# bifurcation/fourq

Hardware: AMD Instinct MI355X
Metric: FourQ scalar-mults/sec (batch, whole node) (higher is better)
Workload: dtype u64

## Files before the change

fourq_amd/build.py:

```python
import json
import os
import re
import shutil
import subprocess
import sys

HERE = os.path.dirname(os.path.abspath(__file__))
SRC_DIR = os.path.join(HERE, "csrc")
LIB_PATH = os.path.join(HERE, "libfourq_amd.so")
RESOURCES_PATH = os.path.join(HERE, "kernel_resources.json")
PLACEMENT_PATH = os.path.join(HERE, "code_placement.json")
SOURCES = ["fourq_amd.hip", "fourq_chain.hip", "fourq_ct_fused.hip", "fourq_ct_chain.hip"]
HEADERS = ["fp127.hip.h", "curve.hip.h", "recode.hip.h", "kernels.hip.h", "pair.hip.h", "ladder_asm.hip.h", "ladder_asm_gfx950.inc", "constants.inc", "pipeline_plan.h", os.path.join("..", "..", "include", "fourq_amd.h")]
HIPCC_FLAGS = ["-O3", "--offload-arch=gfx950", "-std=c++17", "-fPIC", "-fvisibility=hidden", "-Rpass-analysis=kernel-resource-usage"]
PLACE_TOOL = os.path.normpath(os.path.join(HERE, "..", "tools", "asmgen", "place_asm.py"))
LLVM_BIN = "/opt/rocm/lib/llvm/bin"
BUNDLE_TARGETS = "host-x86_64-unknown-linux-gnu,hipv4-amdgcn-amd-amdhsa--gfx950"
BUNDLE_COMPRESS = [] if os.environ.get("FOURQ_BUILD_NO_COMPRESS") == "1" else ["--compress"]

RESOURCE_POLICY = [
    (r"ladder_kernel<\d, 2,", "scratch", lambda v: v == 0, "the two-kernel route's ladders must not spill"),
    (r"ladder_kernel<\d, 2, true", "occupancy", lambda v: v >= 4, "the two-kernel route's DH ladders are sized for 4 waves per SIMD (128 VGPRs)"),
    (r"ladder_kernel<\d, 2, false", "occupancy", lambda v: v >= 2, "the two-kernel route's MUL ladders run the asm bodies at 2 waves per SIMD"),
    (r"ladder_kernel<\d, 1, \w+, \w+, false>", "scratch", lambda v: v == 0, "the fixed-base ladders (MUL and DH) must not spill"),
    (r"ladder_kernel<\d, 1, \w+, \w+, false>", "occupancy", lambda v: v >= 2, "the fixed-base ladders run the asm bodies at 2 waves per SIMD"),
    (r"ladder_kernel<\d, 1, \w+, \w+, true>", "scratch", lambda v: v == 0, "the constant-time fixed-base ladders must not spill"),
    (r"ladder_kernel<\d, 0,", "scratch", lambda v: v == 0, "the fused variable-base kernels must not spill to memory (AGPR copies are fine)"),
    (r"pair_kernel<", "scratch", lambda v: v == 0, "the two-lanes-per-element kernel must not spill"),
    (r"prep_kernel<0, \w+>\(", "occupancy", lambda v: v >= 2, "prep_kernel<ENDO> hides its read-backs behind a second wave per SIMD"),
    (r"mixed_ct_tail_kernel<", "occupancy", lambda v: v >= 2, "the constant-time mixed-batch tail runs the asm bodies at two waves per SIMD"),
    (r"mixed_ct_tail_kernel<", "scratch", lambda v: v == 0, "the constant-time mixed-batch tail must not spill"),
    (r"comb_kernel<true, false>", "scratch", lambda v: v == 0, "the keygen comb of large batches (deferred normalisation) must not touch scratch memory"),
    (r"comb_kernel<false, false>", "scratch", lambda v: v <= 16, "the keygen comb with its inversion in the kernel parks 4 registers around the call: no more than that"),
]


def _hipcc():
    exe = shutil.which("hipcc") or "/opt/rocm/bin/hipcc"
    if not os.path.exists(exe):
        raise RuntimeError("hipcc not found: the FourQ engine needs the ROCm toolchain to build")
    return exe


def _demangle(names):
    filt = shutil.which("c++filt") or "/opt/rocm/lib/llvm/bin/llvm-cxxfilt"
    try:
        out = subprocess.run([filt], input="\n".join(names), capture_output=True, text=True, check=True).stdout.splitlines()
        return [o.replace("fq::(anonymous namespace)::", "").replace("(anonymous namespace)::", "") for o in out]
    except (OSError, subprocess.CalledProcessError):
        return list(names)


_FIELDS = {"TotalSGPRs": "sgprs", "VGPRs": "vgprs", "AGPRs": "agprs", "ScratchSize [bytes/lane]": "scratch",
           "Occupancy [waves/SIMD]": "occupancy", "VGPRs Spill": "vgpr_spills", "SGPRs Spill": "sgpr_spills", "LDS Size [bytes/block]": "lds"}


def parse_resource_remarks(text):
    kernels, cur = {}, None
    for line in text.splitlines():
        m = re.search(r"remark:\s+(Function Name|[A-Za-z ]+(?:\[[^\]]+\])?):\s*(\S+)\s*\[-Rpass-analysis", line)
        if not m:
            continue
        key, val = m.group(1).strip(), m.group(2)
        if key == "Function Name":
            cur = kernels.setdefault(val, {})
        elif cur is not None and key in _FIELDS:
            try:
                cur[_FIELDS[key]] = int(val)
            except ValueError:
                pass
    return kernels


def check_policy(resources):
    bad = []
    for unit, kernels in resources.items():
        for name, f in kernels.items():
            for pattern, field, ok, why in RESOURCE_POLICY:
                if re.search(pattern, name) and field in f and not ok(f[field]):
                    bad.append("%s: %s has %s = %d (%s)" % (unit, name, field, f[field], why))
    return bad


def source_id(extra_flags=()):
    import hashlib
    h = hashlib.sha256()
    for f in [os.path.join(SRC_DIR, f) for f in SOURCES + HEADERS] + [PLACE_TOOL]:
        with open(os.path.normpath(f), "rb") as fh:
            h.update(fh.read())
    h.update(" ".join(list(HIPCC_FLAGS) + list(extra_flags)).encode())
    return h.hexdigest()[:16]


def is_stale():
    if not os.path.exists(LIB_PATH):
        return True
    built = os.path.getmtime(LIB_PATH)
    deps = [os.path.join(SRC_DIR, f) for f in SOURCES + HEADERS] + [PLACE_TOOL]
    return any(os.path.getmtime(os.path.normpath(d)) > built for d in deps)


FASTCODEC_SRC = os.path.join(SRC_DIR, "fastcodec.c")


def fastcodec_path():
    import sysconfig
    return os.path.join(HERE, "_fastcodec" + sysconfig.get_config_var("EXT_SUFFIX"))


def build_fastcodec(force=False, verbose=False):
    import sysconfig
    out = fastcodec_path()
    if not force and os.path.exists(out) and os.path.getmtime(out) >= os.path.getmtime(FASTCODEC_SRC):
        return out
    cc = shutil.which("gcc") or shutil.which("cc")
    if cc is None:
        raise RuntimeError("no C compiler for fourq_amd/csrc/fastcodec.c")
    _run([cc, "-O2", "-shared", "-fPIC", "-Wall", "-I" + sysconfig.get_paths()["include"], "-o", out, FASTCODEC_SRC], verbose)
    return out


def _run(cmd, verbose=False):
    if verbose:
        print(" ".join(cmd), file=sys.stderr)
    proc = subprocess.run(cmd, stdout=subprocess.PIPE, stderr=subprocess.STDOUT, text=True)
    if proc.returncode != 0:
        raise RuntimeError("command failed: %s\n%s" % (" ".join(cmd), "\n".join(l for l in proc.stdout.splitlines() if "remark:" not in l)[-6000:]))
    return proc.stdout


class RegisterOwnershipError(Exception):
    """A kernel reaches a hand-scheduled body whose physical registers lie outside its allocation.  NOT a RuntimeError on purpose: the
    build's fallback for a failed placement detour catches RuntimeError, and this finding must never be swallowed by it -- the plain
    hipcc build of the same sources would carry the same kernel."""


def check_register_ranges(asm_path):
    kernel, highest, alloc, accum = None, {}, {}, {}
    with open(asm_path) as fh:
        for ln in fh:
            m = re.match(r"^(_Z\w+):", ln)
            if m:
                kernel = m.group(1)
                continue
            m = re.match(r"\s*\.amdhsa_kernel\s+(\S+)", ln)
            if m:
                kernel = m.group(1)
                continue
            m = re.match(r"\s*\.amdhsa_next_free_vgpr\s+(\d+)", ln)
            if m and kernel:
                alloc[kernel] = int(m.group(1))
                continue
            m = re.match(r"\s*\.amdhsa_accum_offset\s+(\d+)", ln)
            if m and kernel:
                accum[kernel] = int(m.group(1))
                continue
            t = ln.strip()
            if kernel is None or not t or t[0] in ";.":
                continue
            for a, b in re.findall(r"\bv(\d+)\b|\bv\[\d+:(\d+)\]", t):
                r = int(a or b)
                if r > highest.get(kernel, -1):
                    highest[kernel] = r
    bad = []
    for k, h in highest.items():
        if k not in alloc:
            continue
        owned = min(alloc[k], accum.get(k, alloc[k]))
        if h >= owned:
            bad.append("%s names v%d but owns %d arch VGPRs (next_free_vgpr %d, accum_offset %s)" % (k, h, owned, alloc[k], accum.get(k, "-")))
    if not alloc and highest:
        bad.append("%s: VGPRs are named but no .amdhsa_next_free_vgpr could be parsed -- the listing format changed" % asm_path)
    if bad:
        raise RegisterOwnershipError("a kernel reaches an asm body whose registers it does not own:\n  " + "\n  ".join(bad))


def compile_unit(src, obj, flags, verbose=False, place=True, placement=None):
    src_path = os.path.join(SRC_DIR, src)
    stem = os.path.splitext(obj)[0]
    if not place:
        if placement is not None:
            placement[src] = {"placed": False}
        listing = stem + ".check.s"
        try:
            _run([_hipcc()] + [f for f in flags if not f.startswith("-Rpass")] + ["--cuda-device-only", "-S", "-o", listing, src_path], verbose)
            check_register_ranges(listing)
        finally:
            if os.path.exists(listing):
                os.remove(listing)
        return _run([_hipcc()] + flags + ["-c", "-o", obj, src_path], verbose)
    import importlib.util
    spec = importlib.util.spec_from_file_location("place_asm", PLACE_TOOL)
    place_asm = importlib.util.module_from_spec(spec)
    spec.loader.exec_module(place_asm)
    dev_s, placed_s, dev_o, hsaco, fatbin = stem + ".dev.s", stem + ".placed.s", stem + ".dev.o", stem + ".hsaco", stem + ".hipfb"
    remarks = _run([_hipcc()] + flags + ["--cuda-device-only", "-S", "-o", dev_s, src_path], verbose)
    check_register_ranges(dev_s)
    stats = place_asm.place_file(dev_s, placed_s)
    if placement is not None:
        placement[src] = {"placed": True, "wide_instructions": stats["wide_total"], "at_4_mod_8_before": stats["misaligned_before"],
                          "at_4_mod_8_after": stats["misaligned_after"], "reencoded": stats["promoted"], "nops": stats["nops"],
                          "instructions_compared_with_the_unplaced_object": stats["instructions_compared"]}
    if verbose:
        print("%s: %d of %d 8-byte instructions at 4 mod 8 before placement, %d after" % (
            src, stats["misaligned_before"], stats["wide_total"], stats["misaligned_after"]), file=sys.stderr)
    _run([os.path.join(LLVM_BIN, "clang"), "-x", "assembler", "-target", "amdgcn-amd-amdhsa", "-mcpu=gfx950", "-c", placed_s, "-o", dev_o], verbose)
    _run([os.path.join(LLVM_BIN, "lld"), "-flavor", "gnu", "-m", "elf64_amdgpu", "--no-undefined", "-shared", "-o", hsaco, dev_o], verbose)
    _run([os.path.join(LLVM_BIN, "clang-offload-bundler"), "-type=o", "-bundle-align=4096", "-targets=" + BUNDLE_TARGETS] + BUNDLE_COMPRESS +
         ["-input=/dev/null", "-input=" + hsaco, "-output=" + fatbin], verbose)
    host_flags = [f for f in flags if not f.startswith("-Rpass")]
    _run([_hipcc()] + host_flags + ["--cuda-host-only", "-Xclang", "-fcuda-include-gpubinary", "-Xclang", fatbin, "-c", "-o", obj, src_path], verbose)
    for tmp in (dev_s, placed_s, dev_o, hsaco, fatbin):
        os.remove(tmp)
    return remarks


def build_library(force=False, verbose=False, extra_flags=(), out_path=None):
    if out_path is None:
        try:
            build_fastcodec(force, verbose)
        except Exception as exc:
            print("fourq_amd.build: WARNING -- the tuple codec extension (csrc/fastcodec.c) did not build; fourq_amd.codec falls back to "
                  "its pure-Python conversions (~5 us per element instead of ~0.5):\n%s" % str(exc)[-1500:], file=sys.stderr)
    if out_path is None and not force and not is_stale():
        return LIB_PATH
    from concurrent.futures import ThreadPoolExecutor
    lib_path = out_path or LIB_PATH
    suffix = "" if out_path is None else "." + os.path.splitext(os.path.basename(out_path))[0]
    place = "-DFQ_NO_PLACE=1" not in extra_flags
    flags = HIPCC_FLAGS + list(extra_flags) + ['-DFQ_BUILD_ID="%s"' % source_id(extra_flags)]
    objs = [os.path.join(SRC_DIR, os.path.splitext(src)[0] + suffix + ".o") for src in SOURCES]
    placement = {}
    def one(so):
        try:
            return compile_unit(so[0], so[1], flags, verbose, place, placement)
        except RuntimeError as e:
            if not place:
                raise
            print("fourq_amd.build: code placement of %s failed, building it without the pass:\n%s" % (so[0], str(e)[-1500:]), file=sys.stderr)
            return compile_unit(so[0], so[1], flags, verbose, False, placement)

    with ThreadPoolExecutor(max_workers=len(SOURCES)) as pool:
        outs = list(pool.map(one, zip(SOURCES, objs)))
    resources = {}
    for src, out in zip(SOURCES, outs):
        raw = parse_resource_remarks(out)
        names = list(raw)
        resources[src] = dict(zip(_demangle(names), (raw[n] for n in names)))
    bad = check_policy(resources) if out_path is None and not extra_flags else []
    if bad:
        raise RuntimeError("kernel resource policy violated (fourq_amd/build.py RESOURCE_POLICY):\n  " + "\n  ".join(bad))
    link = [_hipcc(), "--offload-arch=gfx950", "-shared", "-fPIC", "-o", lib_path] + objs
    if verbose:
        print(" ".join(link), file=sys.stderr)
    proc = subprocess.run(link, capture_output=True, text=True)
    if proc.returncode != 0:
        raise RuntimeError("link failed:\n" + proc.stdout + proc.stderr)
    with open(RESOURCES_PATH if out_path is None else lib_path + ".resources.json", "w") as fh:
        json.dump(resources, fh, indent=1, sort_keys=True)
    with open(PLACEMENT_PATH if out_path is None else lib_path + ".placement.json", "w") as fh:
        json.dump(placement, fh, indent=1, sort_keys=True)
    if out_path is not None:
        for obj in objs:
            os.remove(obj)
    return lib_path


if __name__ == "__main__":
    argv = sys.argv[1:]
    out = argv[argv.index("--out") + 1] if "--out" in argv else None
    flags = [a for a in argv if a.startswith("-D") or a.startswith("-m")]
    print(build_library(force="--force" in argv, verbose=True, extra_flags=flags, out_path=os.path.abspath(out) if out else None))
```

fourq_amd/csrc/recode.hip.h:

```cpp
#pragma once
#include "fp127.hip.h"

namespace fq {

typedef unsigned __int128 u128;

FQ_DEV u64 mul_shift256(const u64 a[4], const u64 m[4]) {
    u64 w0, w1, w2, w3, w4;
    u128 t;
    t = (u128)a[0] * m[0];                       w0 = (u64)t;
    t = (u128)a[0] * m[1] + (u64)(t >> 64);      w1 = (u64)t;
    t = (u128)a[0] * m[2] + (u64)(t >> 64);      w2 = (u64)t;
    t = (u128)a[0] * m[3] + (u64)(t >> 64);      w3 = (u64)t; w4 = (u64)(t >> 64);
    t = (u128)a[1] * m[0] + w1;                  w1 = (u64)t;
    t = (u128)a[1] * m[1] + w2 + (u64)(t >> 64); w2 = (u64)t;
    t = (u128)a[1] * m[2] + w3 + (u64)(t >> 64); w3 = (u64)t;
    w4 += a[1] * m[3] + (u64)(t >> 64);
    t = (u128)a[2] * m[0] + w2;                  w2 = (u64)t;
    t = (u128)a[2] * m[1] + w3 + (u64)(t >> 64); w3 = (u64)t;
    w4 += a[2] * m[2] + (u64)(t >> 64);
    t = (u128)a[3] * m[0] + w3;                  w3 = (u64)t;
    w4 += a[3] * m[1] + (u64)(t >> 64);
    (void)w0; (void)w1; (void)w2; (void)w3;
    return w4;
}

FQ_DEV void decompose(const u64 m[4], u64 v[4]) {
    u64 t[4];
#pragma unroll
    for (int i = 0; i < 4; i++) {
        u64 ell[4] = { ELL[i][0], ELL[i][1], ELL[i][2], ELL[i][3] };
        t[i] = mul_shift256(ell, m);
    }
    u64 ac[4], acp[4];
#pragma unroll
    for (int i = 0; i < 4; i++) {
        u64 a = (i == 0) ? m[0] : 0;
#pragma unroll
        for (int j = 0; j < 4; j++) a -= t[j] * BASIS[j][i];
        ac[i] = a + OFFSET_C[i];
        acp[i] = a + OFFSET_CP[i];
    }
    u64 mask = (u64)0 - (ac[0] & 1);
#pragma unroll
    for (int i = 0; i < 4; i++) v[i] = acp[i] ^ (mask & (ac[i] ^ acp[i]));
}

struct EndoDigits {
    u64 sign;
    u64 d[3];
    u32 top;
};
FQ_DEV EndoDigits recode(const u64 vin[4]) {
    EndoDigits r;
    r.sign = vin[0] >> 1;
    u64 v1 = vin[1], v2 = vin[2], v3 = vin[3];
    u64 p1 = 0, p2 = 0, p3 = 0;
    u64 s = r.sign;
#pragma unroll 1
    for (int i = 0; i < 64; i++) {
        u64 nb1 = ~(s >> i) & 1;
        u64 b;
        b = v1 & 1; p1 |= b << i; v1 = (v1 >> 1) + (nb1 & b);
        b = v2 & 1; p2 |= b << i; v2 = (v2 >> 1) + (nb1 & b);
        b = v3 & 1; p3 |= b << i; v3 = (v3 >> 1) + (nb1 & b);
    }
    r.d[0] = p1; r.d[1] = p2; r.d[2] = p3;
    r.top = (u32)(v1 + 2 * v2 + 4 * v3);
    return r;
}
struct EndoNibbles {
    u32 w[8];
    u32 top;
};
FQ_DEV EndoNibbles recode_nibbles(const u64 vin[4]) {
    EndoNibbles r;
    u64 s = vin[0] >> 1;
    u64 v1 = vin[1], v2 = vin[2], v3 = vin[3];
#pragma unroll
    for (int t = 0; t < 8; t++) r.w[t] = 0;
#pragma unroll 1
    for (int k = 0; k < 8; k++) {
        u32 w = 0;
#pragma unroll
        for (int j = 0; j < 8; j++) {
            const u32 nb1 = ~(u32)s & 1;
            s >>= 1;
            const u32 b1 = (u32)v1 & 1, b2 = (u32)v2 & 1, b3 = (u32)v3 & 1;
            v1 = (v1 >> 1) + (nb1 & b1);
            v2 = (v2 >> 1) + (nb1 & b2);
            v3 = (v3 >> 1) + (nb1 & b3);
            w = (w >> 4) | ((b1 | (b2 << 1) | (b3 << 2) | (nb1 << 3)) << 28);
        }
#pragma unroll
        for (int t = 0; t < 7; t++) r.w[t] = r.w[t + 1];
        r.w[7] = w;
    }
    r.top = (u32)(v1 + 2 * v2 + 4 * v3);
    return r;
}
FQ_DEV u32 endo_digit(const EndoDigits& e, int i) {
    return (u32)((e.d[0] >> i) & 1) | ((u32)((e.d[1] >> i) & 1) << 1) | ((u32)((e.d[2] >> i) & 1) << 2);
}
FQ_DEV u32 endo_neg_mask(const EndoDigits& e, int i) {
    return (u32)((e.sign >> i) & 1) - 1u;
}

struct WinScalar {
    u64 r[4];
};
FQ_DEV bool ge256(const u64 a[4], const u64 b[4]) {
    bool ge = true;
#pragma unroll
    for (int i = 0; i < 4; i++) ge = (a[i] == b[i]) ? ge : (a[i] > b[i]);
    return ge;
}
FQ_DEV WinScalar win_reduce(const u64 m[4]) {
    u64 r[4] = { m[0], m[1], m[2], m[3] };
#pragma unroll 1
    for (int k = 10; k >= 0; k--) {
        u64 s[4];
        s[0] = ORDER_N[0] << k;
#pragma unroll
        for (int i = 1; i < 4; i++) s[i] = (ORDER_N[i] << k) | (k ? (ORDER_N[i - 1] >> (64 - k)) : 0);
        u64 keep = ge256(r, s) ? ~(u64)0 : 0;
        u64 borrow = 0;
#pragma unroll
        for (int i = 0; i < 4; i++) {
            u64 si = s[i] & keep;
            u64 d1 = r[i] - si;
            u64 b1 = r[i] < si;
            u64 d2 = d1 - borrow;
            u64 b2 = d1 < borrow;
            r[i] = d2; borrow = b1 | b2;
        }
    }
    u64 addn = (r[0] & 1) ? 0 : ~(u64)0;
    u64 carry = 0;
#pragma unroll
    for (int i = 0; i < 4; i++) {
        u64 ni = ORDER_N[i] & addn;
        u64 s1 = r[i] + ni;
        u64 c1 = s1 < ni;
        u64 s2 = s1 + carry;
        u64 c2 = s2 < carry;
        r[i] = s2; carry = c1 | c2;
    }
    WinScalar w; w.r[0] = r[0]; w.r[1] = r[1]; w.r[2] = r[2]; w.r[3] = r[3];
    return w;
}
FQ_DEV u32 win_code_from_window(u32 w5) {
    u32 w = (w5 & 31) | 1;
    u32 pos = w >> 4;
    u32 ind = ((pos ? w : ~w) & 15) >> 1;
    return (pos << 3) | ind;
}
FQ_DEV u32 win_window(const WinScalar& w, int i) {
    int bit = 4 * i, word = bit >> 6, off = bit & 63;
    u64 lo = (word == 0) ? w.r[0] : (word == 1) ? w.r[1] : (word == 2) ? w.r[2] : w.r[3];
    u64 hi = (word == 0) ? w.r[1] : (word == 1) ? w.r[2] : (word == 2) ? w.r[3] : 0;
    u64 v = lo >> off;
    if (off > 59) v |= hi << (64 - off);
    return (u32)v & 31;
}
FQ_DEV u32 win_top_code(const WinScalar& w) {
    u32 d = (u32)(w.r[3] >> 60) | 1;
    return (1u << 3) | (((d - 1) >> 1) & 7);
}

template <int W_, int V_, int E_> struct CombShape {
    static constexpr int W = W_, V = V_, E = E_, D = V_ * E_, BLOCK_POINTS = 1 << (W_ - 1), POINTS = V_ << (W_ - 1);
    static_assert(W_ * V_ * E_ >= 250 && V_ * E_ <= 64, "comb shape");
};
typedef CombShape<9, 4, 7> CombFast;
typedef CombShape<5, 5, 10> CombScan;
constexpr int COMB_POINTS_ALL = CombFast::POINTS + CombScan::POINTS;
template <typename S> struct CombDigits {
    typedef typename std::conditional<(S::D <= 32), u32, u64>::type plane_t;
    plane_t plane[S::W];
    u32 negate;
};
template <typename S> FQ_DEV CombDigits<S> comb_recode(const u64 m[4]) {
    constexpr int COMB_W = S::W, COMB_D = S::D;
    WinScalar red = win_reduce(m);
    u64 k[4] = { red.r[0], red.r[1], red.r[2], red.r[3] };
    u64 n[4] = { ORDER_N[0], ORDER_N[1], ORDER_N[2], ORDER_N[3] };
    const bool was_even = ge256(k, n);
    u64 twoN[4], alt[4];
    twoN[0] = n[0] << 1; twoN[1] = (n[1] << 1) | (n[0] >> 63); twoN[2] = (n[2] << 1) | (n[1] >> 63); twoN[3] = (n[3] << 1) | (n[2] >> 63);
    u64 borrow = 0;
#pragma unroll
    for (int i = 0; i < 4; i++) {
        u64 d1 = twoN[i] - k[i], b1 = twoN[i] < k[i];
        u64 d2 = d1 - borrow, b2 = d1 < borrow;
        alt[i] = d2; borrow = b1 | b2;
    }
    CombDigits<S> c;
    c.negate = was_even ? ~0u : 0u;
#pragma unroll
    for (int i = 0; i < 4; i++) k[i] = was_even ? alt[i] : k[i];
    const u64 mask_d = (1ull << COMB_D) - 1;
    const u64 sign = ((k[0] >> 1) & (mask_d >> 1)) | (1ull << (COMB_D - 1));
    typedef typename CombDigits<S>::plane_t plane_t;
    c.plane[0] = (plane_t)sign;
    u64 c0 = (k[0] >> COMB_D) | (k[1] << (64 - COMB_D)), c1 = (k[1] >> COMB_D) | (k[2] << (64 - COMB_D));
    u64 c2 = (k[2] >> COMB_D) | (k[3] << (64 - COMB_D)), c3 = k[3] >> COMB_D;
    const plane_t neg = (plane_t)(~sign & mask_d);
#pragma unroll
    for (int r = 1; r < COMB_W; r++) {
        const plane_t low = (plane_t)(c0 & mask_d);
        plane_t T = low;
#pragma unroll 4
        for (int i = 0; i < COMB_D; i++) T = (plane_t)((low + (plane_t)((T & neg) << 1)) & (plane_t)mask_d);
        c.plane[r] = T;
        const u64 up = (u64)(T & neg) << 1, down = (u64)T;
        u64 s0 = c0 + up, cy = s0 < up;
        u64 s1 = c1 + cy; cy = s1 < cy;
        u64 s2 = c2 + cy; cy = s2 < cy;
        u64 s3 = c3 + cy;
        u64 t0 = s0 - down, bw = s0 < down;
        u64 t1 = s1 - bw; bw = s1 < bw;
        u64 t2 = s2 - bw; bw = s2 < bw;
        u64 t3 = s3 - bw;
        c0 = (t0 >> COMB_D) | (t1 << (64 - COMB_D)); c1 = (t1 >> COMB_D) | (t2 << (64 - COMB_D));
        c2 = (t2 >> COMB_D) | (t3 << (64 - COMB_D)); c3 = t3 >> COMB_D;
    }
    return c;
}
template <typename S> FQ_DEV u32 comb_index(const CombDigits<S>& c, int col) {
    u32 idx = 0;
#pragma unroll
    for (int r = 1; r < S::W; r++) idx |= (u32)((c.plane[r] >> col) & 1) << (r - 1);
    return idx;
}
template <typename S> FQ_DEV u32 comb_neg_mask(const CombDigits<S>& c, int col) { return (u32)((c.plane[0] >> col) & 1) - 1u; }
template <typename S> FQ_DEV void comb_point_scalar(u32 t, u64 m[4]) {
    const u32 j = t >> (S::W - 1), u = t & ((1u << (S::W - 1)) - 1);
    m[0] = m[1] = m[2] = m[3] = 0;
    auto set_bit = [&](int bit) { m[bit >> 6] |= 1ull << (bit & 63); };
    set_bit(S::E * j);
    for (int r = 0; r < S::W - 1; r++) if ((u >> r) & 1) set_bit(S::E * j + (r + 1) * S::D);
}

}
```

Baseline: 221.1 million.

## Replace bit-serial endomorphism recoding with closed-form add/xor and bit-matrix transpose

Swaps the 64-iteration bit-by-bit GLV-SAC recoding loop for a closed form. Each digit plane is (v_j + M) xor M, where M is the complemented sign mask, and the top digit comes from the add carry-outs. The nibble-packed variant builds its words with a butterfly bit transpose instead of a serial loop. This removes a long serial dependency chain of per-bit operations in scalar recoding, at the cost of relying on a non-obvious algebraic identity being exactly equivalent.

```diff
diff --git a/fourq_amd/build.py b/fourq_amd/build.py
--- a/fourq_amd/build.py
+++ b/fourq_amd/build.py
@@ -11,7 +11,7 @@
 RESOURCES_PATH = os.path.join(HERE, "kernel_resources.json")
 PLACEMENT_PATH = os.path.join(HERE, "code_placement.json")
 SOURCES = ["fourq_amd.hip", "fourq_chain.hip", "fourq_ct_fused.hip", "fourq_ct_chain.hip"]
-HEADERS = ["fp127.hip.h", "curve.hip.h", "recode.hip.h", "kernels.hip.h", "pair.hip.h", "ladder_asm.hip.h", "ladder_asm_gfx950.inc", "constants.inc", "pipeline_plan.h", os.path.join("..", "..", "include", "fourq_amd.h")]
+HEADERS = ["fp127.hip.h", "curve.hip.h", "recode.hip.h", "recode_closed.h", "kernels.hip.h", "pair.hip.h", "ladder_asm.hip.h", "ladder_asm_gfx950.inc", "constants.inc", "pipeline_plan.h", os.path.join("..", "..", "include", "fourq_amd.h")]
 HIPCC_FLAGS = ["-O3", "--offload-arch=gfx950", "-std=c++17", "-fPIC", "-fvisibility=hidden", "-Rpass-analysis=kernel-resource-usage"]
 PLACE_TOOL = os.path.normpath(os.path.join(HERE, "..", "tools", "asmgen", "place_asm.py"))
 LLVM_BIN = "/opt/rocm/lib/llvm/bin"
diff --git a/fourq_amd/csrc/recode.hip.h b/fourq_amd/csrc/recode.hip.h
--- a/fourq_amd/csrc/recode.hip.h
+++ b/fourq_amd/csrc/recode.hip.h
@@ -1,5 +1,6 @@
 #pragma once
 #include "fp127.hip.h"
+#include "recode_closed.h"
 
 namespace fq {
 
@@ -52,21 +53,11 @@
     u32 top;
 };
 FQ_DEV EndoDigits recode(const u64 vin[4]) {
+    const fq_rc::Planes p = fq_rc::planes(vin);
     EndoDigits r;
-    r.sign = vin[0] >> 1;
-    u64 v1 = vin[1], v2 = vin[2], v3 = vin[3];
-    u64 p1 = 0, p2 = 0, p3 = 0;
-    u64 s = r.sign;
-#pragma unroll 1
-    for (int i = 0; i < 64; i++) {
-        u64 nb1 = ~(s >> i) & 1;
-        u64 b;
-        b = v1 & 1; p1 |= b << i; v1 = (v1 >> 1) + (nb1 & b);
-        b = v2 & 1; p2 |= b << i; v2 = (v2 >> 1) + (nb1 & b);
-        b = v3 & 1; p3 |= b << i; v3 = (v3 >> 1) + (nb1 & b);
-    }
-    r.d[0] = p1; r.d[1] = p2; r.d[2] = p3;
-    r.top = (u32)(v1 + 2 * v2 + 4 * v3);
+    r.sign = ~p.sub;
+    r.d[0] = p.p[0]; r.d[1] = p.p[1]; r.d[2] = p.p[2];
+    r.top = p.top;
     return r;
 }
 struct EndoNibbles {
@@ -75,28 +66,7 @@
 };
 FQ_DEV EndoNibbles recode_nibbles(const u64 vin[4]) {
     EndoNibbles r;
-    u64 s = vin[0] >> 1;
-    u64 v1 = vin[1], v2 = vin[2], v3 = vin[3];
-#pragma unroll
-    for (int t = 0; t < 8; t++) r.w[t] = 0;
-#pragma unroll 1
-    for (int k = 0; k < 8; k++) {
-        u32 w = 0;
-#pragma unroll
-        for (int j = 0; j < 8; j++) {
-            const u32 nb1 = ~(u32)s & 1;
-            s >>= 1;
-            const u32 b1 = (u32)v1 & 1, b2 = (u32)v2 & 1, b3 = (u32)v3 & 1;
-            v1 = (v1 >> 1) + (nb1 & b1);
-            v2 = (v2 >> 1) + (nb1 & b2);
-            v3 = (v3 >> 1) + (nb1 & b3);
-            w = (w >> 4) | ((b1 | (b2 << 1) | (b3 << 2) | (nb1 << 3)) << 28);
-        }
-#pragma unroll
-        for (int t = 0; t < 7; t++) r.w[t] = r.w[t + 1];
-        r.w[7] = w;
-    }
-    r.top = (u32)(v1 + 2 * v2 + 4 * v3);
+    fq_rc::nibbles(vin, r.w, &r.top);
     return r;
 }
 FQ_DEV u32 endo_digit(const EndoDigits& e, int i) {
diff --git a/fourq_amd/csrc/recode_closed.h b/fourq_amd/csrc/recode_closed.h
--- /dev/null
+++ b/fourq_amd/csrc/recode_closed.h
@@ -0,0 +1,70 @@
+#pragma once
+#include <stdint.h>
+
+#if defined(__HIP__) || defined(__HIPCC__)
+#define FQ_RC_FN __host__ __device__ __forceinline__
+#define FQ_RC_UNROLL _Pragma("unroll")
+#else
+#define FQ_RC_FN inline
+#define FQ_RC_UNROLL _Pragma("GCC unroll 8")
+#endif
+
+namespace fq_rc {
+
+struct Planes {
+    uint64_t p[3];
+    uint64_t sub;
+    uint32_t top;
+};
+
+FQ_RC_FN uint32_t carry_out(uint64_t a, uint64_t b, uint64_t s) {
+    return (uint32_t)((((a & b) | ((a | b) & ~s)) >> 63));
+}
+
+FQ_RC_FN Planes planes(const uint64_t v[4]) {
+    Planes r;
+    const uint64_t M = ~(v[0] >> 1);
+    r.sub = M;
+    uint32_t top = 0;
+FQ_RC_UNROLL
+    for (int j = 0; j < 3; j++) {
+        const uint64_t s = v[j + 1] + M;
+        r.p[j] = s ^ M;
+        top |= carry_out(v[j + 1], M, s) << j;
+    }
+    r.top = top;
+    return r;
+}
+
+FQ_RC_FN void exchange(uint32_t& lo, uint32_t& hi, uint32_t mask, int delta) {
+    const uint32_t l = lo, h = hi;
+    lo = (l & ~mask) | ((h << delta) & mask);
+    hi = (h & mask) | ((l >> delta) & ~mask);
+}
+FQ_RC_FN void nibbles(const uint64_t v[4], uint32_t w[8], uint32_t* top) {
+    const Planes r = planes(v);
+    uint32_t x[8];
+FQ_RC_UNROLL
+    for (int q = 0; q < 4; q++) {
+        const uint64_t plane = q < 3 ? r.p[q] : r.sub;
+        x[q] = (uint32_t)plane;
+        x[q + 4] = (uint32_t)(plane >> 32);
+    }
+FQ_RC_UNROLL
+    for (int i = 0; i < 8; i += 2) {
+        exchange(x[i], x[i + 1], 0xAAAAAAAAu, 1);
+        exchange(x[i], x[i + 1], 0xF0F0F0F0u, 4);
+        exchange(x[i], x[i + 1], 0xFFFF0000u, 16);
+    }
+FQ_RC_UNROLL
+    for (int j = 0; j < 4; j++) {
+        const int i = (j & 1) | ((j & 2) << 1);
+        exchange(x[i], x[i + 2], 0xCCCCCCCCu, 2);
+        exchange(x[i], x[i + 2], 0xFF00FF00u, 8);
+    }
+FQ_RC_UNROLL
+    for (int t = 0; t < 8; t++) w[t] = x[(t & 4) | ((t & 1) << 1) | ((t >> 1) & 1)];
+    *top = r.top;
+}
+
+}
```

New measurement: 223.2 million (median of 6 runs). Within noise of the previous version (+1.0%).
